# jerryli27/TwinGAN

Hardware: AMD Instinct MI355X
Metric: training images/sec (G+D step) at 256×256 final stage, 1/2/4/8 MI355X (higher is better)
Workload: dtype bf16; 1 GPU; TwinGAN 256x256 stage, batch 16 per GPU (configs[3]): E/G/2xD max_ch 256, UNet + per-domain instance norm + pixel norm, WGAN-GP, Adam; 1 step = G apply + D apply; global_batch=16, batch_per_gpu=16, parallelism=dp1, launch=hipGraph replay

## Files before the change

twingan_amd/csrc/reduce.hip:

```cpp
#include "tg_common.h"
#include "../../include/twingan_hip_optim.h"
#include "../../include/twingan_hip_summary.h"

namespace {

constexpr int MB_NMAX = 16;
template <typename T, int V>
struct alignas(sizeof(T) * V) MbVec {
  T e[V];
  __device__ __forceinline__ float get(int i) const { return (float)e[i]; }
  __device__ __forceinline__ void set(int i, float x) { e[i] = (T)x; }
};
template <typename T> constexpr int mb_v() { return 8 / (int)sizeof(T); }
template <typename T, int V> __device__ __forceinline__ MbVec<T, V> mb_ld(const T* p) {
  return *reinterpret_cast<const MbVec<T, V>*>(p);
}
template <typename T, int V> __device__ __forceinline__ void mb_st(T* p, const MbVec<T, V>& v) {
  *reinterpret_cast<MbVec<T, V>*>(p) = v;
}
template <typename T, int V>
__device__ __forceinline__ void mb_load_samples(const T* __restrict__ x, int n, int P, int p, MbVec<T, V> (&xv)[MB_NMAX]) {
#pragma unroll
  for (int i = 0; i < MB_NMAX; ++i) xv[i] = mb_ld<T, V>(x + (int64_t)(i < n ? i : n - 1) * P + p);
}


template <typename T, int U = 4>
__device__ __forceinline__ void mb_copy_with_stat(const T* __restrict__ src, T* __restrict__ out, int64_t nvec, int c,
                                                  int cpad, float val) {
  constexpr int V = Vec16<T>::N;
  const int cvp = cpad / V;
  for (int64_t i0 = threadIdx.x; i0 < nvec; i0 += (int64_t)blockDim.x * U) {
    Vec16<T> o[U];
#pragma unroll
    for (int u = 0; u < U; ++u) {
      int64_t i = i0 + (int64_t)u * blockDim.x;
      i = i < nvec ? i : nvec - 1;
      const int cb = (int)(i % cvp) * V;
      const int64_t px = i / cvp;
      if (cb < c) {
        o[u] = ldv(src + px * c + cb);
      } else {
#pragma unroll
        for (int j = 0; j < V; ++j) o[u].set(j, (cb + j == c) ? val : 0.f);
      }
    }
#pragma unroll
    for (int u = 0; u < U; ++u) {
      const int64_t i = i0 + (int64_t)u * blockDim.x;
      if (i < nvec) stv(out + (i / cvp) * cpad + (int)(i % cvp) * V, o[u]);
    }
  }
}

template <typename T>
__global__ __launch_bounds__(1024) void mbstd_fwd_kernel(const T* __restrict__ x, T* __restrict__ out,
                                                         float* __restrict__ stat, int n, int hw, int c, int cpad,
                                                         float eps) {
  __shared__ float red[16];
  const int P = hw * c;
  x += (int64_t)blockIdx.x * n * P;
  out += (int64_t)blockIdx.x * n * hw * cpad;
  if (stat) stat += blockIdx.x;
  float acc = 0.f;
  constexpr int V = mb_v<T>();
  if (P % V == 0 && n <= 32) {
    for (int p = threadIdx.x * V; p < P; p += blockDim.x * V) {
      float mu[V], var[V];
#pragma unroll
      for (int j = 0; j < V; ++j) mu[j] = var[j] = 0.f;
      if (n <= MB_NMAX) {
        MbVec<T, V> xs[MB_NMAX];
        mb_load_samples<T, V>(x, n, P, p, xs);
#pragma unroll
        for (int i = 0; i < MB_NMAX; ++i)
          if (i < n) {
#pragma unroll
            for (int j = 0; j < V; ++j) mu[j] += xs[i].get(j);
          }
#pragma unroll
        for (int j = 0; j < V; ++j) mu[j] /= (float)n;
#pragma unroll
        for (int i = 0; i < MB_NMAX; ++i)
          if (i < n) {
#pragma unroll
            for (int j = 0; j < V; ++j) {
              const float d = xs[i].get(j) - mu[j];
              var[j] = fmaf(d, d, var[j]);
            }
          }
      } else {
        for (int i = 0; i < n; ++i) {
          const MbVec<T, V> xv = mb_ld<T, V>(x + (int64_t)i * P + p);
#pragma unroll
          for (int j = 0; j < V; ++j) mu[j] += xv.get(j);
        }
#pragma unroll
        for (int j = 0; j < V; ++j) mu[j] /= (float)n;
        for (int i = 0; i < n; ++i) {
          const MbVec<T, V> xv = mb_ld<T, V>(x + (int64_t)i * P + p);
#pragma unroll
          for (int j = 0; j < V; ++j) {
            const float d = xv.get(j) - mu[j];
            var[j] = fmaf(d, d, var[j]);
          }
        }
      }
#pragma unroll
      for (int j = 0; j < V; ++j) acc += sqrtf(var[j] / (float)n + eps);
    }
  } else {
    for (int p = threadIdx.x; p < P; p += blockDim.x) {
      float mu = 0.f;
      for (int i = 0; i < n; ++i) mu += ld(x + (int64_t)i * P + p);
      mu /= (float)n;
      float var = 0.f;
      for (int i = 0; i < n; ++i) {
        const float d = ld(x + (int64_t)i * P + p) - mu;
        var = fmaf(d, d, var);
      }
      acc += sqrtf(var / (float)n + eps);
    }
  }
  const float val = block_sum(acc, red) / (float)P;
  if (threadIdx.x == 0 && stat) stat[0] = val;
  const int64_t total = (int64_t)n * hw * cpad;
  constexpr int V16 = Vec16<T>::N;
  if (c % V16 == 0 && cpad % V16 == 0) {
    mb_copy_with_stat<T, 9>(x, out, total / V16, c, cpad, val);
  } else {
    for (int64_t i = threadIdx.x; i < total; i += blockDim.x) {
      const int ch = (int)(i % cpad);
      const int64_t px = i / cpad;
      float v = 0.f;
      if (ch < c)
        v = ld(x + px * c + ch);
      else if (ch == c)
        v = val;
      st(out + i, v);
    }
  }
}

template <typename T>
__global__ __launch_bounds__(256) void mbstd_bwd_kernel(const T* __restrict__ gout, const T* __restrict__ x,
                                                        T* __restrict__ gx, int n, int hw, int c, int cpad, float eps) {
  __shared__ float red[16];
  const int P = hw * c;
  gout += (int64_t)blockIdx.x * n * hw * cpad;
  x += (int64_t)blockIdx.x * n * P;
  gx += (int64_t)blockIdx.x * n * P;
  constexpr int V = mb_v<T>();
  const bool fast = c % V == 0 && cpad % V == 0 && n <= MB_NMAX;
  MbVec<T, V> xs[MB_NMAX], gs[MB_NMAX];
  const int pstep = gridDim.y * blockDim.x * V;
  const int pfirst = (blockIdx.y * blockDim.x + threadIdx.x) * V;
  if (fast) {
    const int p = pfirst < P ? pfirst : 0;
    const int px = p / c, ch = p - px * c;
    mb_load_samples<T, V>(x, n, P, p, xs);
#pragma unroll
    for (int i = 0; i < MB_NMAX; ++i) gs[i] = mb_ld<T, V>(gout + ((int64_t)(i < n ? i : n - 1) * hw + px) * cpad + ch);
  }
  float acc = 0.f;
  for (int i = threadIdx.x; i < n * hw; i += blockDim.x) acc += ld(gout + (int64_t)i * cpad + c);
  const float G = block_sum(acc, red);
  if (fast) {
    for (int p = pfirst; p < P; p += pstep) {
      float mu[V], var[V], k[V];
      if (p != pfirst) {
        const int px = p / c, ch = p - px * c;
        mb_load_samples<T, V>(x, n, P, p, xs);
#pragma unroll
        for (int i = 0; i < MB_NMAX; ++i) gs[i] = mb_ld<T, V>(gout + ((int64_t)(i < n ? i : n - 1) * hw + px) * cpad + ch);
      }
#pragma unroll
      for (int j = 0; j < V; ++j) mu[j] = var[j] = 0.f;
#pragma unroll
      for (int i = 0; i < MB_NMAX; ++i)
        if (i < n) {
#pragma unroll
          for (int j = 0; j < V; ++j) mu[j] += xs[i].get(j);
        }
#pragma unroll
// ... 47 lines not shown
        const MbVec<T, V> xv = mb_ld<T, V>(x + (int64_t)i * P + p);
        const MbVec<T, V> gv = mb_ld<T, V>(gout + ((int64_t)i * hw + px) * cpad + ch);
        MbVec<T, V> o;
#pragma unroll
        for (int j = 0; j < V; ++j) o.set(j, gv.get(j) + k[j] * (xv.get(j) - mu[j]));
        mb_st<T, V>(gx + (int64_t)i * P + p, o);
      }
    }
    return;
  }
  for (int p = blockIdx.y * blockDim.x + threadIdx.x; p < P; p += gridDim.y * blockDim.x) {
    float mu = 0.f;
    for (int i = 0; i < n; ++i) mu += ld(x + (int64_t)i * P + p);
    mu /= (float)n;
    float var = 0.f;
    for (int i = 0; i < n; ++i) {
      const float d = ld(x + (int64_t)i * P + p) - mu;
      var = fmaf(d, d, var);
    }
    const float sigma = sqrtf(var / (float)n + eps);
    const float k = G / ((float)n * sigma * (float)P);
    const int px = p / c, ch = p - px * c;
    for (int i = 0; i < n; ++i) {
      const float d = ld(x + (int64_t)i * P + p) - mu;
      st(gx + (int64_t)i * P + p, ld(gout + ((int64_t)i * hw + px) * cpad + ch) + k * d);
    }
  }
}

template <typename T, int NTHR>
__global__ __launch_bounds__(NTHR) void mbstd_bwd_bwd_kernel(const T* __restrict__ v, const T* __restrict__ gout,
                                                            const T* __restrict__ x, T* __restrict__ ggout,
                                                            T* __restrict__ gx2, int n, int hw, int c, int cpad,
                                                            float eps) {
  __shared__ float red[16];
  const int P = hw * c;
  v += (int64_t)blockIdx.x * n * P;
  gout += (int64_t)blockIdx.x * n * hw * cpad;
  x += (int64_t)blockIdx.x * n * P;
  if (ggout) ggout += (int64_t)blockIdx.x * n * hw * cpad;
  if (gx2) gx2 += (int64_t)blockIdx.x * n * P;
  constexpr int V = mb_v<T>();
  const bool fast = P % V == 0 && n <= MB_NMAX;
  MbVec<T, V> xs[MB_NMAX], vs[MB_NMAX];
  const int pfirst = threadIdx.x * V;
  if (fast) {
    mb_load_samples<T, V>(x, n, P, pfirst < P ? pfirst : 0, xs);
    mb_load_samples<T, V>(v, n, P, pfirst < P ? pfirst : 0, vs);
  }
  float acc = 0.f;
  for (int i = threadIdx.x; i < n * hw; i += blockDim.x) acc += ld(gout + (int64_t)i * cpad + c);
  const float G = block_sum(acc, red);
  float tacc = 0.f;
  if (fast) {
    for (int p = pfirst; p < P; p += blockDim.x * V) {
      if (p != pfirst) {
        mb_load_samples<T, V>(x, n, P, p, xs);
        mb_load_samples<T, V>(v, n, P, p, vs);
      }
      float mu[V], vm[V], var[V], vc[V], sigma[V];
#pragma unroll
      for (int j = 0; j < V; ++j) mu[j] = vm[j] = var[j] = vc[j] = 0.f;
#pragma unroll
      for (int i = 0; i < MB_NMAX; ++i)
        if (i < n) {
#pragma unroll
          for (int j = 0; j < V; ++j) {
            mu[j] += xs[i].get(j);
            vm[j] += vs[i].get(j);
          }
        }
#pragma unroll
      for (int j = 0; j < V; ++j) {
        mu[j] /= (float)n;
        vm[j] /= (float)n;
      }
#pragma unroll
      for (int i = 0; i < MB_NMAX; ++i)
        if (i < n) {
#pragma unroll
          for (int j = 0; j < V; ++j) {
            const float d = xs[i].get(j) - mu[j];
            var[j] = fmaf(d, d, var[j]);
            vc[j] = fmaf(vs[i].get(j), d, vc[j]);
          }
        }
#pragma unroll
      for (int j = 0; j < V; ++j) {
        sigma[j] = sqrtf(var[j] / (float)n + eps);
        tacc += vc[j] / ((float)n * sigma[j] * (float)P);
      }
      if (gx2) {
        const float k = G / ((float)n * (float)P);
        float is[V], cf[V];
#pragma unroll
        for (int j = 0; j < V; ++j) {
          is[j] = 1.f / sigma[j];
          cf[j] = vc[j] * is[j] * is[j] * is[j] / (float)n;
        }
#pragma unroll
        for (int i = 0; i < MB_NMAX; ++i)
          if (i < n) {
            MbVec<T, V> o;
#pragma unroll
            for (int j = 0; j < V; ++j) {
              const float d = xs[i].get(j) - mu[j];
              o.set(j, k * ((vs[i].get(j) - vm[j]) * is[j] - cf[j] * d));
            }
            mb_st<T, V>(gx2 + (int64_t)i * P + p, o);
          }
      }
    }
  }
  for (int p = threadIdx.x; p < P && !fast; p += blockDim.x) {
    float mu = 0.f, vm = 0.f;
    for (int i = 0; i < n; ++i) {
      mu += ld(x + (int64_t)i * P + p);
      vm += ld(v + (int64_t)i * P + p);
    }
    mu /= (float)n;
    vm /= (float)n;
    float var = 0.f, vc = 0.f;
    for (int i = 0; i < n; ++i) {
      const float d = ld(x + (int64_t)i * P + p) - mu;
      var = fmaf(d, d, var);
      vc = fmaf(ld(v + (int64_t)i * P + p), d, vc);
    }
    const float sigma = sqrtf(var / (float)n + eps);
    tacc += vc / ((float)n * sigma * (float)P);
    if (gx2) {
      const float k = G / ((float)n * (float)P);
      for (int i = 0; i < n; ++i) {
        const float d = ld(x + (int64_t)i * P + p) - mu;
        const float vi = ld(v + (int64_t)i * P + p);
        st(gx2 + (int64_t)i * P + p, k * ((vi - vm) / sigma - vc * d / ((float)n * sigma * sigma * sigma)));
      }
    }
  }
  const float Tt = block_sum(tacc, red);
  if (ggout) {
    const int64_t total = (int64_t)n * hw * cpad;
    constexpr int V16 = Vec16<T>::N;
    if (c % V16 == 0 && cpad % V16 == 0) {
      mb_copy_with_stat<T, 9>(v, ggout, total / V16, c, cpad, Tt);
    } else {
      for (int64_t i = threadIdx.x; i < total; i += blockDim.x) {
        const int ch = (int)(i % cpad);
        const int64_t px = i / cpad;
        float o = 0.f;
        if (ch < c)
          o = ld(v + px * c + ch);
        else if (ch == c)
          o = Tt;
        st(ggout + i, o);
      }
    }
  }
}

template <typename T, int MODE, bool PART = false>
__global__ void sum_kernel(const T* __restrict__ x, const T* __restrict__ y, float* __restrict__ out, int64_t numel,
                           float scale, int direct = 0, int vec = 1) {
  __shared__ float red[8];
  constexpr int V = Vec16<T>::N;
  const int64_t nvec = vec ? numel / V : 0, stride = (int64_t)gridDim.x * blockDim.x;
  float acc = 0.f;
  for (int64_t i = (int64_t)blockIdx.x * blockDim.x + threadIdx.x; i < nvec; i += stride) {
    Vec16<T> a = ldv(x + i * V);
    if (MODE == 0) {
#pragma unroll
      for (int j = 0; j < V; ++j) acc += a.get(j);
    } else {
      Vec16<T> b = ldv(y + i * V);
#pragma unroll
      for (int j = 0; j < V; ++j) acc += fabsf(a.get(j) - b.get(j));
    }
  }
  for (int64_t i = nvec * V + (int64_t)blockIdx.x * blockDim.x + threadIdx.x; i < numel; i += stride)
    acc += MODE == 0 ? ld(x + i) : fabsf(ld(x + i) - ld(y + i));
  const float tot = block_sum(acc, red);
  if (threadIdx.x == 0) {
    if constexpr (PART) out[blockIdx.x] = tot;
    else if (direct) out[0] = tot * scale;
    else atomicAdd(out, tot * scale);
  }
}

__global__ void ordered_scalar_sum_kernel(const float* __restrict__ part, int n, float* __restrict__ out, float scale,
                                          int accumulate) {
  if (blockIdx.x || threadIdx.x) return;
  float t = 0.f;
  for (int i = 0; i < n; ++i) t += part[i];
  out[0] = accumulate ? out[0] + t * scale : t * scale;
}

__device__ __forceinline__ int nonfinite_bits(float x) {
  return (__builtin_bit_cast(uint32_t, x) & 0x7f800000u) == 0x7f800000u;
}
__device__ __forceinline__ float nan_where_nonfinite(float grad, float arg) {
  return nonfinite_bits(arg) ? __builtin_nanf("") : grad;
}

template <typename T>
__global__ void abs_diff_bwd_kernel(const T* __restrict__ a, const T* __restrict__ b, const float* __restrict__ gscale,
                                    T* __restrict__ ga, T* __restrict__ gb, int64_t numel, float scale) {
  const float g = (gscale ? gscale[0] : 1.f) * scale;
  for (int64_t i = (int64_t)blockIdx.x * blockDim.x + threadIdx.x; i < numel; i += (int64_t)gridDim.x * blockDim.x) {
    const float d = ld(a + i) - ld(b + i);
    const float s = nan_where_nonfinite(d > 0.f ? g : (d < 0.f ? -g : 0.f), d);
    if (ga) st(ga + i, s);
    if (gb) st(gb + i, -s);
  }
}

template <typename T>
__global__ void sample_sumsq_kernel(const T* __restrict__ x, float* __restrict__ out, int64_t per, int vec) {
  __shared__ float red[8];
  constexpr int V = Vec16<T>::N;
  const T* base = x + (int64_t)blockIdx.y * per;
  const int64_t nvec = vec ? per / V : 0, stride = (int64_t)gridDim.x * blockDim.x;
  float acc = 0.f;
  for (int64_t i = (int64_t)blockIdx.x * blockDim.x + threadIdx.x; i < nvec; i += stride) {
    Vec16<T> a = ldv(base + i * V);
#pragma unroll
    for (int j = 0; j < V; ++j) acc = fmaf(a.get(j), a.get(j), acc);
  }
  for (int64_t i = nvec * V + (int64_t)blockIdx.x * blockDim.x + threadIdx.x; i < per; i += stride) {
    const float a = ld(base + i);
    acc = fmaf(a, a, acc);
  }
  const float tot = block_sum(acc, red);
  if (threadIdx.x == 0) atomicAdd(out + blockIdx.y, tot);
}

__global__ void gp_penalty_kernel(const float* __restrict__ ss, float* __restrict__ loss, float* __restrict__ coef,
                                  int batch, float lambda) {
  __shared__ float red[8];
  float acc = 0.f;
  for (int b = threadIdx.x; b < batch; b += blockDim.x) {
    const float slope = sqrtf(ss[b]);
    const float d = slope - 1.f;
    acc += d * d;
    if (coef) coef[b] = slope == 0.f ? 0.f : lambda * 2.f * d / (slope * (float)batch);
  }
  const float tot = block_sum(acc, red);
  if (threadIdx.x == 0 && loss) loss[0] = lambda * tot / (float)batch;
}

__device__ __forceinline__ float pred_loss_f(float x, int mode, float a, float b) {
  if (mode == 1) {
    const float z = a + b * x;
    return z < 0.f ? 0.f : z;
  }
  if (mode == 2) return fmaxf(x, 0.f) - x * a + log1pf(expf(-fabsf(x)));
  if (mode == 3) return x * x;
  return x;
}
__device__ __forceinline__ float pred_loss_df_finite(float x, int mode, float a, float b) {
  if (mode == 1) return (a + b * x) > 0.f ? b : 0.f;
  if (mode == 2) return 1.f / (1.f + expf(-x)) - a;
  if (mode == 3) return 2.f * x;
  return 1.f;
}
__device__ __forceinline__ float pred_loss_df(float x, int mode, float a, float b) {
  return nan_where_nonfinite(pred_loss_df_finite(x, mode, a, b), x);
}
__global__ void pred_loss_fwd_kernel(const float* __restrict__ x, float* __restrict__ out, int n, int mode, float a,
                                     float b, float scale, int accumulate) {
  __shared__ float red[8];
  float acc = 0.f;
  for (int i = threadIdx.x; i < n; i += blockDim.x) acc += pred_loss_f(x[i], mode, a, b);
  const float tot = block_sum(acc, red);
  if (threadIdx.x == 0) out[0] = (accumulate ? out[0] : 0.f) + scale * tot;
}
__global__ void pred_loss_bwd_kernel(const float* __restrict__ x, const float* __restrict__ gscale, float* __restrict__ gx,
                                     int n, int mode, float a, float b, float scale) {
  const float g = (gscale ? gscale[0] : 1.f) * scale;
  for (int i = blockIdx.x * blockDim.x + threadIdx.x; i < n; i += gridDim.x * blockDim.x)
// ... 56 lines not shown
  for (int r = 0; r < b; ++r) {
    float dot = 0.f, se = 0.f, sp = 0.f;
    for (int c = threadIdx.x; c < d; c += 256) {
      const float x = e[(size_t)r * d + c], y = p[(size_t)r * d + c];
      dot = fmaf(x, y, dot);
      se = fmaf(x, x, se);
      sp = fmaf(y, y, sp);
    }
    dot = block_sum(dot, red);
    se = block_sum(se, red);
    sp = block_sum(sp, red);
    tot += 1.f - dot * rsqrtf(fmaxf(se, 1e-12f)) * rsqrtf(fmaxf(sp, 1e-12f));
  }
  if (threadIdx.x == 0) out[0] = tot * scale;
}

__global__ __launch_bounds__(256) void cosine_distance_bwd_kernel(const float* __restrict__ e, const float* __restrict__ p,
                                                                  const float* __restrict__ gscale, float* __restrict__ gp,
                                                                  int d, float scale) {
  __shared__ float red[4];
  const int r = blockIdx.x;
  float dot = 0.f, se = 0.f, sp = 0.f;
  for (int c = threadIdx.x; c < d; c += 256) {
    const float x = e[(size_t)r * d + c], y = p[(size_t)r * d + c];
    dot = fmaf(x, y, dot);
    se = fmaf(x, x, se);
    sp = fmaf(y, y, sp);
  }
  dot = block_sum(dot, red);
  se = block_sum(se, red);
  sp = block_sum(sp, red);
  const float ie = rsqrtf(fmaxf(se, 1e-12f)), ip = rsqrtf(fmaxf(sp, 1e-12f));
  const float cosv = dot * ie * ip, k = -scale * gscale[0];
  const bool clamped = sp < 1e-12f;
  for (int c = threadIdx.x; c < d; c += 256) {
    const float eh = e[(size_t)r * d + c] * ie, ph = p[(size_t)r * d + c] * ip;
    gp[(size_t)r * d + c] = k * (clamped ? eh * ip : (eh - ph * cosv) * ip);
  }
}

__global__ void var_from_sums_kernel(const float* __restrict__ s1, const float* __restrict__ ss, float* __restrict__ out,
                                     int batch, float inv_numel) {
  __shared__ float red[8];
  float acc = 0.f;
  for (int i = threadIdx.x; i < batch; i += blockDim.x) acc += ss[i];
  const float tot = block_sum(acc, red);
  if (threadIdx.x == 0) {
    const float m = s1[0] * inv_numel;
    const float v = tot * inv_numel - m * m;
    out[0] = v < 0.f ? 0.f : v;
  }
}

template <typename T>
__global__ void fc_fwd_kernel(const T* __restrict__ x, const float* __restrict__ w, const float* __restrict__ b,
                              float* __restrict__ y, int m, int n, int k) {
  const int64_t total = (int64_t)m * n;
  const int lane = threadIdx.x & 63;
  const int64_t w0 = ((int64_t)blockIdx.x * blockDim.x + threadIdx.x) >> 6, nw = ((int64_t)gridDim.x * blockDim.x) >> 6;
  for (int64_t i = w0; i < total; i += nw) {
    const int col = (int)(i % n), row = (int)(i / n);
    float acc = 0.f;
    for (int kk = lane; kk < k; kk += 64) acc = fmaf(ld(x + (int64_t)row * k + kk), w[(int64_t)kk * n + col], acc);
#pragma unroll
    for (int o = 32; o > 0; o >>= 1) acc += __shfl_xor(acc, o, 64);
    if (lane == 0) y[i] = acc + (b ? b[col] : 0.f);
  }
}
template <typename T>
__global__ void fc_bwd_kernel(const T* __restrict__ x, const float* __restrict__ w, const float* __restrict__ g,
                              T* __restrict__ gx, float* __restrict__ gw, float* __restrict__ gb, int m, int n, int k,
                              int acc_w, int acc_b) {
  const int kk = blockIdx.x * blockDim.x + threadIdx.x;
  if (kk < k) {
    for (int row = 0; gx && row < m; ++row) {
      float a = 0.f;
      for (int col = 0; col < n; ++col) a = fmaf(g[(int64_t)row * n + col], w[(int64_t)kk * n + col], a);
      st(gx + (int64_t)row * k + kk, a);
    }
    for (int col = 0; gw && col < n; ++col) {
      float a = 0.f;
      for (int row = 0; row < m; ++row) a = fmaf(ld(x + (int64_t)row * k + kk), g[(int64_t)row * n + col], a);
      gw[(int64_t)kk * n + col] = (acc_w ? gw[(int64_t)kk * n + col] : 0.f) + a;
    }
  }
  if (gb && kk < n) {
    float a = 0.f;
    for (int row = 0; row < m; ++row) a += g[(int64_t)row * n + kk];
    gb[kk] = (acc_b ? gb[kk] : 0.f) + a;
  }
}

__global__ void small_gemm_kernel(const float* __restrict__ a, const float* __restrict__ b, const float* __restrict__ bias,
                                  float* __restrict__ c, int m, int n, int k, int ta, int tb, int accumulate) {
  const int64_t total = (int64_t)m * n;
  for (int64_t i = (int64_t)blockIdx.x * blockDim.x + threadIdx.x; i < total; i += (int64_t)gridDim.x * blockDim.x) {
    const int col = (int)(i % n), row = (int)(i / n);
    float acc = 0.f;
    for (int kk = 0; kk < k; ++kk) {
      const float av = ta ? a[(int64_t)kk * m + row] : a[(int64_t)row * k + kk];
      const float bv = tb ? b[(int64_t)col * k + kk] : b[(int64_t)kk * n + col];
      acc = fmaf(av, bv, acc);
    }
    if (bias) acc += bias[col];
    c[i] = (accumulate ? c[i] : 0.f) + acc;
  }
}

__global__ void small_gemm_wave_kernel(const float* __restrict__ a, const float* __restrict__ b,
                                       const float* __restrict__ bias, float* __restrict__ c, int m, int n, int k, int ta,
                                       int tb, int accumulate) {
  const int64_t total = (int64_t)m * n;
  const int lane = threadIdx.x & 63;
  const int64_t w0 = ((int64_t)blockIdx.x * blockDim.x + threadIdx.x) >> 6, nw = ((int64_t)gridDim.x * blockDim.x) >> 6;
  for (int64_t i = w0; i < total; i += nw) {
    const int col = (int)(i % n), row = (int)(i / n);
    float acc = 0.f;
    for (int kk = lane; kk < k; kk += 64) {
      const float av = ta ? a[(int64_t)kk * m + row] : a[(int64_t)row * k + kk];
      const float bv = tb ? b[(int64_t)col * k + kk] : b[(int64_t)kk * n + col];
      acc = fmaf(av, bv, acc);
    }
    acc = wave_sum(acc);
    if (lane == 0) {
      if (bias) acc += bias[col];
      c[i] = (accumulate ? c[i] : 0.f) + acc;
    }
  }
}

__device__ __forceinline__ float adam_element(float th, float gi, float& m, float& v, float lr_t, float b1, float b2, float eps) {
  const float mi = fmaf(b1, m, (1.f - b1) * gi);
  const float vi = fmaf(b2, v, (1.f - b2) * gi * gi);
  m = mi;
  v = vi;
  return th - lr_t * mi / (sqrtf(vi) + eps);
}

__device__ __forceinline__ float ema_element(float avg, float var, float w) { return fmaf(-(avg - var), w, avg); }

template <bool VEC>
__device__ __forceinline__ void ema_span(float* __restrict__ avg, const float* __restrict__ var, int64_t numel, float w,
// ... 373 lines not shown
  }
  if ((tid & 63) == 0) red[tid >> 6] = SummaryPartial{acc.sum, acc.sumsq, acc.mn, acc.mx, acc.num, acc.zeros, acc.nonfinite, 0u};
  __syncthreads();
  if (tid == 0) {
    SummaryPartial r = red[0];
    for (int w = 1; w < SUM_THREADS / TG_WAVE; ++w) {
      r.sum += red[w].sum;
      r.sumsq += red[w].sumsq;
      r.mn = fminf(r.mn, red[w].mn);
      r.mx = fmaxf(r.mx, red[w].mx);
      r.num += red[w].num;
      r.zeros += red[w].zeros;
      r.nonfinite += red[w].nonfinite;
    }
    partials[b] = r;
  }
  uint32_t* dst = buckets + (size_t)j.out * TG_SUMMARY_BUCKETS;
  for (int i = tid; i < TG_SUMMARY_BUCKETS; i += SUM_THREADS) {
    const unsigned n = hist[i];
    if (n) atomicAdd(&dst[i], n);
  }
}

__global__ __launch_bounds__(64) void summary_finish_kernel(const SummaryJob* __restrict__ jobs, int njobs, int nout,
                                                            const SummaryPartial* __restrict__ partials,
                                                            TgSummaryStats* __restrict__ stats) {
  const int k = blockIdx.x * 64 + threadIdx.x;
  if (k >= njobs) return;
  const SummaryJob j = jobs[k];
  if (j.out >= nout) return;
  TgSummaryStats r{0.0, 0.0, SUM_FLT_MAX, -SUM_FLT_MAX, 0u, 0u, 0u, 0u};
  for (int b = j.block_begin; b < j.block_end; ++b) {
    const SummaryPartial p = partials[b];
    r.sum += p.sum;
    r.sum_squares += p.sumsq;
    r.min = fminf(r.min, p.mn);
    r.max = fmaxf(r.max, p.mx);
    r.num += p.num;
    r.zeros += p.zeros;
    r.nonfinite += p.nonfinite;
  }
  stats[j.out] = r;
}

}

extern "C" {

int tg_mbstd_fwd(const void* x, void* out, float* stat, int n, int groups, int hw, int c, int cpad, float eps, int dtype,
                 void* stream) {
  TG_CHECK(x && out && n > 0 && hw > 0 && c > 0 && cpad > c, TG_EINVAL, "tg_mbstd_fwd: bad arguments (cpad must exceed c)");
  TG_CHECK(groups > 0 && n % groups == 0, TG_EINVAL, "tg_mbstd_fwd: n (%d) not divisible by groups (%d)", n, groups);
  TG_DISPATCH_DTYPE(dtype, "tg_mbstd_fwd", {
    hipLaunchKernelGGL(mbstd_fwd_kernel<T>, dim3(groups), dim3(1024), 0, (hipStream_t)stream, (const T*)x, (T*)out, stat,
                       n / groups, hw, c, cpad, eps);
  });
  TG_LAUNCH_CHECK("tg_mbstd_fwd");
  return TG_OK;
}

int tg_mbstd_bwd(const void* gout, const void* x, void* gx, int n, int groups, int hw, int c, int cpad, float eps,
                 int dtype, void* stream) {
  TG_CHECK(gout && x && gx && n > 0 && hw > 0 && c > 0 && cpad > c, TG_EINVAL, "tg_mbstd_bwd: bad arguments");
  TG_CHECK(groups > 0 && n % groups == 0, TG_EINVAL, "tg_mbstd_bwd: n (%d) not divisible by groups (%d)", n, groups);
  TG_DISPATCH_DTYPE(dtype, "tg_mbstd_bwd", {
    int nsplit = (hw * c / mb_v<T>() + 255) / 256;
    if (nsplit < 1) nsplit = 1;
    if (nsplit > 8) nsplit = 8;
    hipLaunchKernelGGL(mbstd_bwd_kernel<T>, dim3(groups, nsplit), dim3(256), 0, (hipStream_t)stream, (const T*)gout, (const T*)x,
                       (T*)gx, n / groups, hw, c, cpad, eps);
  });
  TG_LAUNCH_CHECK("tg_mbstd_bwd");
  return TG_OK;
}

int tg_mbstd_bwd_bwd(const void* v, const void* gout, const void* x, void* ggout, void* gx2, int n, int groups, int hw, int c,
                     int cpad, float eps, int dtype, void* stream) {
  TG_CHECK(v && gout && x && n > 0 && hw > 0 && c > 0 && cpad > c, TG_EINVAL, "tg_mbstd_bwd_bwd: bad arguments");
  TG_CHECK(groups > 0 && n % groups == 0, TG_EINVAL, "tg_mbstd_bwd_bwd: n (%d) not divisible by groups (%d)", n, groups);
  TG_DISPATCH_DTYPE(dtype, "tg_mbstd_bwd_bwd", {
    constexpr int NTHR = sizeof(T) == 4 ? 512 : 1024;
    hipLaunchKernelGGL((mbstd_bwd_bwd_kernel<T, NTHR>), dim3(groups), dim3(NTHR), 0, (hipStream_t)stream, (const T*)v,
                       (const T*)gout, (const T*)x, (T*)ggout, (T*)gx2, n / groups, hw, c, cpad, eps);
  });
  TG_LAUNCH_CHECK("tg_mbstd_bwd_bwd");
  return TG_OK;
}

static int zero_unless(float* p, size_t bytes, int accumulate, hipStream_t s, const char* who) {
  if (!accumulate) return tg_zero_async(p, bytes, nullptr, 0, s);
  return TG_OK;
}

int tg_sum(const void* x, float* out, int64_t numel, float scale, int accumulate, int dtype, void* stream) {
  TG_CHECK(x && out && numel > 0, TG_EINVAL, "tg_sum: bad arguments");
  hipStream_t s = (hipStream_t)stream;
  TG_DISPATCH_DTYPE(dtype, "tg_sum", {
    const int blocks = exact_grid<T>() ? 1 : tg_grid_for(numel / Vec16<T>::N + 1, 256, 1024);
    const int direct = (blocks == 1 && !accumulate) ? 1 : 0;
    if (!direct) {
      int rc = zero_unless(out, sizeof(float), accumulate, s, "tg_sum");
      if (rc) return rc;
    }
    hipLaunchKernelGGL((sum_kernel<T, 0>), dim3(blocks), dim3(256), 0, s, (const T*)x, (const T*)nullptr, out, numel, scale, direct,
                       tg_aligned16(x));
  });
  TG_LAUNCH_CHECK("tg_sum");
  return TG_OK;
}

int tg_abs_diff_sum(const void* a, const void* b, float* out, int64_t numel, float scale, int accumulate, int dtype,
                    void* stream) {
  TG_CHECK(a && b && out && numel > 0, TG_EINVAL, "tg_abs_diff_sum: bad arguments");
  hipStream_t s = (hipStream_t)stream;
  TG_DISPATCH_DTYPE(dtype, "tg_abs_diff_sum", {
    const int blocks = exact_grid<T>() ? 1 : tg_grid_for(numel / Vec16<T>::N + 1, 256, 1024);
    const int direct = (blocks == 1 && !accumulate) ? 1 : 0;
    if (!direct) {
      int rc = zero_unless(out, sizeof(float), accumulate, s, "tg_abs_diff_sum");
      if (rc) return rc;
    }
    hipLaunchKernelGGL((sum_kernel<T, 1>), dim3(blocks), dim3(256), 0, s, (const T*)a, (const T*)b, out, numel, scale, direct,
                       tg_aligned16(a) && tg_aligned16(b));
  });
  TG_LAUNCH_CHECK("tg_abs_diff_sum");
  return TG_OK;
}

int tg_sum_ordered(const void* x, const void* y_or_null, float* out, int64_t numel, float scale, int accumulate, float* ws,
                   size_t ws_floats, int dtype, void* stream) {
  TG_CHECK(x && out && ws && ws_floats >= 1 && numel > 0, TG_EINVAL, "tg_sum_ordered: bad arguments");
  hipStream_t s = (hipStream_t)stream;
  int blocks = 0;
  TG_DISPATCH_DTYPE(dtype, "tg_sum_ordered", {
    blocks = tg_grid_for(numel / Vec16<T>::N + 1, 256, 512);
    if ((size_t)blocks > ws_floats) blocks = (int)ws_floats;
    if (y_or_null)
      hipLaunchKernelGGL((sum_kernel<T, 1, true>), dim3(blocks), dim3(256), 0, s, (const T*)x, (const T*)y_or_null, ws, numel, 1.f, 0,
                         tg_aligned16(x) && tg_aligned16(y_or_null));
    else
      hipLaunchKernelGGL((sum_kernel<T, 0, true>), dim3(blocks), dim3(256), 0, s, (const T*)x, (const T*)nullptr, ws, numel, 1.f, 0,
                         tg_aligned16(x));
  });
  hipLaunchKernelGGL(ordered_scalar_sum_kernel, dim3(1), dim3(64), 0, s, ws, blocks, out, scale, accumulate);
  TG_LAUNCH_CHECK("tg_sum_ordered");
  return TG_OK;
}

int tg_abs_diff_bwd(const void* a, const void* b, const float* gscale, void* ga, void* gb, int64_t numel, float scale,
                    int dtype, void* stream) {
  TG_CHECK(a && b && numel > 0 && (ga || gb), TG_EINVAL, "tg_abs_diff_bwd: bad arguments");
  TG_DISPATCH_DTYPE(dtype, "tg_abs_diff_bwd", {
    hipLaunchKernelGGL(abs_diff_bwd_kernel<T>, dim3(tg_grid_for(numel, 256)), dim3(256), 0, (hipStream_t)stream,
                       (const T*)a, (const T*)b, gscale, (T*)ga, (T*)gb, numel, scale);
  });
  TG_LAUNCH_CHECK("tg_abs_diff_bwd");
  return TG_OK;
}

int tg_sample_sumsq(const void* x, float* out, int batch, int64_t per, int dtype, void* stream) {
  TG_CHECK(x && out && batch > 0 && per > 0, TG_EINVAL, "tg_sample_sumsq: bad arguments");
  hipStream_t s = (hipStream_t)stream;
  int rc = zero_unless(out, (size_t)batch * sizeof(float), 0, s, "tg_sample_sumsq");
  if (rc) return rc;
  TG_DISPATCH_DTYPE(dtype, "tg_sample_sumsq", {
    const int chunks = exact_grid<T>() ? 1 : tg_grid_for(per / Vec16<T>::N + 1, 256, 64);
    const int vec = tg_aligned16(x) && (batch == 1 || per % Vec16<T>::N == 0);
    hipLaunchKernelGGL(sample_sumsq_kernel<T>, dim3(chunks, batch), dim3(256), 0, s, (const T*)x, out, per, vec);
  });
  TG_LAUNCH_CHECK("tg_sample_sumsq");
  return TG_OK;
}

int tg_gp_penalty(const float* sumsq, float* loss, float* coef, int batch, float lambda, void* stream) {
  TG_CHECK(sumsq && batch > 0, TG_EINVAL, "tg_gp_penalty: bad arguments");
  hipLaunchKernelGGL(gp_penalty_kernel, dim3(1), dim3(256), 0, (hipStream_t)stream, sumsq, loss, coef, batch, lambda);
  TG_LAUNCH_CHECK("tg_gp_penalty");
  return TG_OK;
}

int tg_pred_loss_fwd(const float* x, float* out, int n, int mode, float a, float b, float scale, int accumulate,
                     void* stream) {
  TG_CHECK(x && out && n > 0 && mode >= 0 && mode <= 3, TG_EINVAL, "tg_pred_loss_fwd: bad arguments");
  hipLaunchKernelGGL(pred_loss_fwd_kernel, dim3(1), dim3(256), 0, (hipStream_t)stream, x, out, n, mode, a, b, scale,
                     accumulate);
  TG_LAUNCH_CHECK("tg_pred_loss_fwd");
  return TG_OK;
}

int tg_pred_loss_bwd(const float* x, const float* gscale, float* gx, int n, int mode, float a, float b, float scale,
                     void* stream) {
  TG_CHECK(x && gx && n > 0 && mode >= 0 && mode <= 3, TG_EINVAL, "tg_pred_loss_bwd: bad arguments");
  hipLaunchKernelGGL(pred_loss_bwd_kernel, dim3(tg_grid_for(n, 256)), dim3(256), 0, (hipStream_t)stream, x, gscale, gx, n,
                     mode, a, b, scale);
  TG_LAUNCH_CHECK("tg_pred_loss_bwd");
  return TG_OK;
}

int tg_pred_losses_fwd(const float* pred, int group_size, int groups, const TgPredJob* jobs, int njobs, float* terms, int nterms,
                       void* stream) {
  TG_CHECK(pred && jobs && terms && group_size > 0 && groups > 0 && njobs > 0 && njobs <= PRED_MAX_JOBS && nterms > 0 &&
               nterms <= PRED_MAX_TERMS, TG_EINVAL, "tg_pred_losses_fwd: bad arguments (at most %d jobs, %d terms)", PRED_MAX_JOBS,
           PRED_MAX_TERMS);
  PredJobs pj;
  pj.n = njobs;
  for (int j = 0; j < njobs; ++j) {
    TG_CHECK(jobs[j].group >= 0 && jobs[j].group < groups && jobs[j].term >= 0 && jobs[j].term < nterms && jobs[j].mode >= 0 &&
                 jobs[j].mode <= 3, TG_EINVAL, "tg_pred_losses_fwd: job %d out of range", j);
    pj.j[j] = jobs[j];
  }
  hipLaunchKernelGGL(pred_losses_fwd_kernel, dim3(1), dim3(256), 0, (hipStream_t)stream, pred, group_size, pj, terms, nterms);
  TG_LAUNCH_CHECK("tg_pred_losses_fwd");
  return TG_OK;
}

int tg_pred_losses_bwd(const float* pred, int group_size, int groups, const TgPredJob* jobs, int njobs, const float* const* gterms,
                       int nterms, float* gpred, void* stream) {
  TG_CHECK(pred && jobs && gterms && gpred && group_size > 0 && groups > 0 && njobs > 0 && njobs <= PRED_MAX_JOBS && nterms > 0 &&
               nterms <= PRED_MAX_TERMS, TG_EINVAL, "tg_pred_losses_bwd: bad arguments");
// ... 29 lines not shown
                           void* stream) {
  TG_CHECK(expected && embedding && out && batch > 0 && dim > 0, TG_EINVAL, "tg_cosine_distance_fwd: bad arguments");
  hipLaunchKernelGGL(cosine_distance_fwd_kernel, dim3(1), dim3(256), 0, (hipStream_t)stream, expected, embedding, out, batch,
                     dim, weight / (float)batch);
  TG_LAUNCH_CHECK("tg_cosine_distance_fwd");
  return TG_OK;
}

int tg_cosine_distance_bwd(const float* expected, const float* embedding, const float* gscale, float* g_embedding, int batch,
                           int dim, float weight, void* stream) {
  TG_CHECK(expected && embedding && gscale && g_embedding && batch > 0 && dim > 0, TG_EINVAL,
           "tg_cosine_distance_bwd: bad arguments");
  hipLaunchKernelGGL(cosine_distance_bwd_kernel, dim3(batch), dim3(256), 0, (hipStream_t)stream, expected, embedding, gscale,
                     g_embedding, dim, weight / (float)batch);
  TG_LAUNCH_CHECK("tg_cosine_distance_bwd");
  return TG_OK;
}

int tg_var_from_sums(const float* sum, const float* sample_sumsq, float* out, int batch, int64_t numel, void* stream) {
  TG_CHECK(sum && sample_sumsq && out && batch > 0 && numel > 0, TG_EINVAL, "tg_var_from_sums: bad arguments");
  hipLaunchKernelGGL(var_from_sums_kernel, dim3(1), dim3(256), 0, (hipStream_t)stream, sum, sample_sumsq, out, batch,
                     1.0f / (float)numel);
  TG_LAUNCH_CHECK("tg_var_from_sums");
  return TG_OK;
}

int tg_small_gemm(const float* a, const float* b, const float* bias, float* c, int m, int n, int k, int ta, int tb,
                  int accumulate, void* stream) {
  TG_CHECK(a && b && c && m > 0 && n > 0 && k > 0, TG_EINVAL, "tg_small_gemm: bad arguments");
  if (k >= 32 && (int64_t)m * n <= 4096)
    hipLaunchKernelGGL(small_gemm_wave_kernel, dim3(tg_grid_for((int64_t)m * n * 64, 256)), dim3(256), 0,
                       (hipStream_t)stream, a, b, bias, c, m, n, k, ta, tb, accumulate);
  else
    hipLaunchKernelGGL(small_gemm_kernel, dim3(tg_grid_for((int64_t)m * n, 256)), dim3(256), 0, (hipStream_t)stream, a, b,
                       bias, c, m, n, k, ta, tb, accumulate);
  TG_LAUNCH_CHECK("tg_small_gemm");
  return TG_OK;
}

int tg_fc_fwd(const void* x, const float* w, const float* bias, float* y, int m, int n, int k, int dtype, void* stream) {
  TG_CHECK(x && w && y && m > 0 && n > 0 && k > 0, TG_EINVAL, "tg_fc_fwd: bad arguments");
  TG_DISPATCH_DTYPE(dtype, "tg_fc_fwd", {
    hipLaunchKernelGGL(fc_fwd_kernel<T>, dim3(tg_grid_for((int64_t)m * n * 64, 256)), dim3(256), 0, (hipStream_t)stream,
                       (const T*)x, w, bias, y, m, n, k);
  });
  TG_LAUNCH_CHECK("tg_fc_fwd");
  return TG_OK;
}

int tg_fc_bwd(const void* x, const float* w, const float* g, void* gx, float* gw, float* gb, int m, int n, int k, int acc_w,
              int acc_b, int dtype, void* stream) {
  TG_CHECK(x && w && g && (gx || gw || gb) && m > 0 && n > 0 && k > 0 && n <= k, TG_EINVAL, "tg_fc_bwd: bad arguments");
  TG_DISPATCH_DTYPE(dtype, "tg_fc_bwd", {
    hipLaunchKernelGGL(fc_bwd_kernel<T>, dim3(tg_grid_for(k, 64)), dim3(64), 0, (hipStream_t)stream, (const T*)x, w, g, (T*)gx,
                       gw, gb, m, n, k, acc_w, acc_b);
  });
  TG_LAUNCH_CHECK("tg_fc_bwd");
  return TG_OK;
}

int tg_adam_step(float* theta, const float* grad, float* m, float* v, void* theta_bf16, int64_t numel, float lr_t,
                 const float* lr_t_dev, float beta1, float beta2, float eps, float grad_scale, void* stream) {
  TG_CHECK(theta && grad && m && v && numel > 0, TG_EINVAL, "tg_adam_step: bad arguments");
  ApplyArgs a{theta, grad, m, v, numel, {lr_t, beta1, beta2, eps}, grad_scale};
  a.lr_t_dev = lr_t_dev;
  a.shadow = (bf16*)theta_bf16;
  return launch_apply<TG_OPT_ADAM>(a, stream, "tg_adam_step");
}

int tg_adam_ema_step(float* theta, const float* grad, float* m, float* v, float* avg, int64_t numel, const float* lr_t_dev,
                     float beta1, float beta2, float eps, float grad_scale, const float* w_dev, void* stream) {
  TG_CHECK(theta && grad && m && v && avg && lr_t_dev && w_dev, TG_EINVAL, "tg_adam_ema_step: null pointer");
  TG_CHECK(numel > 0, TG_EINVAL, "tg_adam_ema_step: numel must be positive (got %lld)", (long long)numel);
  return launch_apply<TG_OPT_ADAM>({theta, grad, m, v, numel, {0.f, beta1, beta2, eps}, grad_scale, nullptr, avg, w_dev, lr_t_dev},
                                   stream, "tg_adam_ema_step");
}

int tg_ema_update(float* avg, const float* var, int64_t numel, const float* w_dev, void* stream) {
  TG_CHECK(avg && var && w_dev, TG_EINVAL, "tg_ema_update: null pointer");
  TG_CHECK(numel > 0, TG_EINVAL, "tg_ema_update: numel must be positive (got %lld)", (long long)numel);
  if (tg_aligned16(avg) && tg_aligned16(var))
    hipLaunchKernelGGL(ema_kernel<true>, dim3(tg_grid_for((numel + 3) / 4, 256)), dim3(256), 0, (hipStream_t)stream, avg, var,
                       numel, w_dev);
  else
    hipLaunchKernelGGL(ema_kernel<false>, dim3(tg_grid_for(numel, 256)), dim3(256), 0, (hipStream_t)stream, avg, var, numel,
                       w_dev);
  TG_LAUNCH_CHECK("tg_ema_update");
  return TG_OK;
}

size_t tg_ema_table_bytes(int njobs) { return (size_t)(njobs > 0 ? njobs : 0) * sizeof(EmaJob); }

int tg_ema_table_fill(float* avg, const float* var, int64_t numel, int job, void* table_host, int32_t* total_blocks) {
  TG_CHECK(avg && var && table_host && total_blocks && job >= 0, TG_EINVAL, "tg_ema_table_fill: bad arguments");
  TG_CHECK(numel > 0, TG_EINVAL, "tg_ema_table_fill: numel must be positive (got %lld)", (long long)numel);
  const int64_t blocks = (numel + EMA_EPB - 1) / EMA_EPB;
  TG_CHECK(*total_blocks >= 0 && *total_blocks + blocks <= 0x7fffffff, TG_EINVAL, "tg_ema_table_fill: grid too large");
  EmaJob j;
  j.avg = avg;
  j.var = var;
  j.numel = numel;
  j.block_begin = *total_blocks;
  j.block_end = j.block_begin + (int)blocks;
  *total_blocks = j.block_end;
  ((EmaJob*)table_host)[job] = j;
  return TG_OK;
}
// ... 181 lines not shown
```

Baseline: 1049 images/sec.

## Split mbstd copies across grid.y, unroll reductions, and parallelize fc backward per element

Minibatch-stddev forward and double-backward kernels now launch extra blocks along grid.y. Each block redundantly recomputes the statistics and handles only a slice of the padded output copy and the per-sample gradient writes, which spreads a single-block-per-group copy over more CUs. The copy helper uses 32-bit index math with a smaller unroll. The sum and sum-of-squares reductions get an 8-way load unroll with fewer atomic blocks. The fc backward kernel is rewritten to give one thread per output element across the gx, gw and gb segments instead of one thread per k column looping over everything, with register-unrolled inner loops. The cost is duplicated stat computation per y-block and more launched blocks.

```diff
diff --git a/twingan_amd/csrc/reduce.hip b/twingan_amd/csrc/reduce.hip
--- a/twingan_amd/csrc/reduce.hip
+++ b/twingan_amd/csrc/reduce.hip
@@ -25,32 +25,45 @@
 }
 
 
-template <typename T, int U = 4>
+constexpr int MB_COPY_U = 3;
+template <typename T, int U, typename I>
+__device__ __forceinline__ void mb_copy_with_stat_as(const T* __restrict__ src, T* __restrict__ out, I nvec, int c,
+                                                     int cpad, float val) {
+  constexpr int V = Vec16<T>::N;
+  const I cvp = (I)(cpad / V), step = (I)gridDim.y * blockDim.x;
+  for (I i0 = (I)blockIdx.y * blockDim.x + threadIdx.x; i0 < nvec; i0 += step * U) {
+    Vec16<T> o[U];
+    I px[U];
+    int cb[U];
+#pragma unroll
+    for (int u = 0; u < U; ++u) {
+      I i = i0 + (I)u * step;
+      i = i < nvec ? i : nvec - 1;
+      px[u] = i / cvp;
+      cb[u] = (int)(i - px[u] * cvp) * V;
+      if (cb[u] < c) {
+        o[u] = ldv(src + (int64_t)px[u] * c + cb[u]);
+      } else {
+#pragma unroll
+        for (int j = 0; j < V; ++j) o[u].set(j, (cb[u] + j == c) ? val : 0.f);
+      }
+    }
+#pragma unroll
+    for (int u = 0; u < U; ++u)
+      if (i0 + (I)u * step < nvec) stv(out + (int64_t)px[u] * cpad + cb[u], o[u]);
+  }
+}
+template <typename T, int U = MB_COPY_U>
 __device__ __forceinline__ void mb_copy_with_stat(const T* __restrict__ src, T* __restrict__ out, int64_t nvec, int c,
                                                   int cpad, float val) {
-  constexpr int V = Vec16<T>::N;
-  const int cvp = cpad / V;
-  for (int64_t i0 = threadIdx.x; i0 < nvec; i0 += (int64_t)blockDim.x * U) {
-    Vec16<T> o[U];
-#pragma unroll
-    for (int u = 0; u < U; ++u) {
-      int64_t i = i0 + (int64_t)u * blockDim.x;
-      i = i < nvec ? i : nvec - 1;
-      const int cb = (int)(i % cvp) * V;
-      const int64_t px = i / cvp;
-      if (cb < c) {
-        o[u] = ldv(src + px * c + cb);
-      } else {
-#pragma unroll
-        for (int j = 0; j < V; ++j) o[u].set(j, (cb + j == c) ? val : 0.f);
-      }
-    }
-#pragma unroll
-    for (int u = 0; u < U; ++u) {
-      const int64_t i = i0 + (int64_t)u * blockDim.x;
-      if (i < nvec) stv(out + (i / cvp) * cpad + (int)(i % cvp) * V, o[u]);
-    }
-  }
+  if (nvec < (int64_t)1 << 30) mb_copy_with_stat_as<T, U, uint32_t>(src, out, (uint32_t)nvec, c, cpad, val);
+  else mb_copy_with_stat_as<T, U, int64_t>(src, out, nvec, c, cpad, val);
+}
+template <typename T> static int mb_copy_split(int n_per_group, int hw, int cpad, int threads) {
+  const int64_t nvec = (int64_t)n_per_group * hw * cpad / Vec16<T>::N;
+  const int64_t per = (int64_t)threads * MB_COPY_U;
+  const int64_t ny = (nvec + per - 1) / per;
+  return ny < 1 ? 1 : ny > 8 ? 8 : (int)ny;
 }
 
 template <typename T>
@@ -123,13 +136,13 @@
     }
   }
   const float val = block_sum(acc, red) / (float)P;
-  if (threadIdx.x == 0 && stat) stat[0] = val;
+  if (threadIdx.x == 0 && blockIdx.y == 0 && stat) stat[0] = val;
   const int64_t total = (int64_t)n * hw * cpad;
   constexpr int V16 = Vec16<T>::N;
   if (c % V16 == 0 && cpad % V16 == 0) {
-    mb_copy_with_stat<T, 9>(x, out, total / V16, c, cpad, val);
+    mb_copy_with_stat<T>(x, out, total / V16, c, cpad, val);
   } else {
-    for (int64_t i = threadIdx.x; i < total; i += blockDim.x) {
+    for (int64_t i = (int64_t)blockIdx.y * blockDim.x + threadIdx.x; i < total; i += (int64_t)gridDim.y * blockDim.x) {
       const int ch = (int)(i % cpad);
       const int64_t px = i / cpad;
       float v = 0.f;
@@ -283,6 +296,8 @@
   for (int i = threadIdx.x; i < n * hw; i += blockDim.x) acc += ld(gout + (int64_t)i * cpad + c);
   const float G = block_sum(acc, red);
   float tacc = 0.f;
+  unsigned mine = 0;
+  for (int i = blockIdx.y; i < MB_NMAX; i += gridDim.y) mine |= 1u << i;
   if (fast) {
     for (int p = pfirst; p < P; p += blockDim.x * V) {
       if (p != pfirst) {
@@ -331,7 +346,7 @@
         }
 #pragma unroll
         for (int i = 0; i < MB_NMAX; ++i)
-          if (i < n) {
+          if (i < n && (mine >> i & 1u)) {
             MbVec<T, V> o;
 #pragma unroll
             for (int j = 0; j < V; ++j) {
@@ -361,7 +376,7 @@
     tacc += vc / ((float)n * sigma * (float)P);
     if (gx2) {
       const float k = G / ((float)n * (float)P);
-      for (int i = 0; i < n; ++i) {
+      for (int i = blockIdx.y; i < n; i += gridDim.y) {
         const float d = ld(x + (int64_t)i * P + p) - mu;
         const float vi = ld(v + (int64_t)i * P + p);
         st(gx2 + (int64_t)i * P + p, k * ((vi - vm) / sigma - vc * d / ((float)n * sigma * sigma * sigma)));
@@ -373,9 +388,9 @@
     const int64_t total = (int64_t)n * hw * cpad;
     constexpr int V16 = Vec16<T>::N;
     if (c % V16 == 0 && cpad % V16 == 0) {
-      mb_copy_with_stat<T, 9>(v, ggout, total / V16, c, cpad, Tt);
+      mb_copy_with_stat<T>(v, ggout, total / V16, c, cpad, Tt);
     } else {
-      for (int64_t i = threadIdx.x; i < total; i += blockDim.x) {
+      for (int64_t i = (int64_t)blockIdx.y * blockDim.x + threadIdx.x; i < total; i += (int64_t)gridDim.y * blockDim.x) {
         const int ch = (int)(i % cpad);
         const int64_t px = i / cpad;
         float o = 0.f;
@@ -389,6 +404,8 @@
   }
 }
 
+constexpr int RED_U = 8;
+constexpr int RED_ATOMIC_BLOCKS = 256;
 template <typename T, int MODE, bool PART = false>
 __global__ void sum_kernel(const T* __restrict__ x, const T* __restrict__ y, float* __restrict__ out, int64_t numel,
                            float scale, int direct = 0, int vec = 1) {
@@ -396,16 +413,20 @@
   constexpr int V = Vec16<T>::N;
   const int64_t nvec = vec ? numel / V : 0, stride = (int64_t)gridDim.x * blockDim.x;
   float acc = 0.f;
-  for (int64_t i = (int64_t)blockIdx.x * blockDim.x + threadIdx.x; i < nvec; i += stride) {
-    Vec16<T> a = ldv(x + i * V);
-    if (MODE == 0) {
-#pragma unroll
-      for (int j = 0; j < V; ++j) acc += a.get(j);
-    } else {
-      Vec16<T> b = ldv(y + i * V);
-#pragma unroll
-      for (int j = 0; j < V; ++j) acc += fabsf(a.get(j) - b.get(j));
-    }
+  for (int64_t i0 = (int64_t)blockIdx.x * blockDim.x + threadIdx.x; i0 < nvec; i0 += stride * RED_U) {
+    Vec16<T> a[RED_U], b[RED_U];
+#pragma unroll
+    for (int u = 0; u < RED_U; ++u) {
+      const int64_t i = i0 + u * stride < nvec ? i0 + u * stride : nvec - 1;
+      a[u] = ldv(x + i * V);
+      if (MODE != 0) b[u] = ldv(y + i * V);
+    }
+#pragma unroll
+    for (int u = 0; u < RED_U; ++u)
+      if (i0 + u * stride < nvec) {
+#pragma unroll
+        for (int j = 0; j < V; ++j) acc += MODE == 0 ? a[u].get(j) : fabsf(a[u].get(j) - b[u].get(j));
+      }
   }
   for (int64_t i = nvec * V + (int64_t)blockIdx.x * blockDim.x + threadIdx.x; i < numel; i += stride)
     acc += MODE == 0 ? ld(x + i) : fabsf(ld(x + i) - ld(y + i));
@@ -451,10 +472,16 @@
   const T* base = x + (int64_t)blockIdx.y * per;
   const int64_t nvec = vec ? per / V : 0, stride = (int64_t)gridDim.x * blockDim.x;
   float acc = 0.f;
-  for (int64_t i = (int64_t)blockIdx.x * blockDim.x + threadIdx.x; i < nvec; i += stride) {
-    Vec16<T> a = ldv(base + i * V);
-#pragma unroll
-    for (int j = 0; j < V; ++j) acc = fmaf(a.get(j), a.get(j), acc);
+  for (int64_t i0 = (int64_t)blockIdx.x * blockDim.x + threadIdx.x; i0 < nvec; i0 += stride * RED_U) {
+    Vec16<T> a[RED_U];
+#pragma unroll
+    for (int u = 0; u < RED_U; ++u) a[u] = ldv(base + (i0 + u * stride < nvec ? i0 + u * stride : nvec - 1) * V);
+#pragma unroll
+    for (int u = 0; u < RED_U; ++u)
+      if (i0 + u * stride < nvec) {
+#pragma unroll
+        for (int j = 0; j < V; ++j) acc = fmaf(a[u].get(j), a[u].get(j), acc);
+      }
   }
   for (int64_t i = nvec * V + (int64_t)blockIdx.x * blockDim.x + threadIdx.x; i < per; i += stride) {
     const float a = ld(base + i);
@@ -617,6 +644,7 @@
   }
 }
 
+constexpr int FC_U = 16;
 template <typename T>
 __global__ void fc_fwd_kernel(const T* __restrict__ x, const float* __restrict__ w, const float* __restrict__ b,
                               float* __restrict__ y, int m, int n, int k) {
@@ -636,23 +664,67 @@
 __global__ void fc_bwd_kernel(const T* __restrict__ x, const float* __restrict__ w, const float* __restrict__ g,
                               T* __restrict__ gx, float* __restrict__ gw, float* __restrict__ gb, int m, int n, int k,
                               int acc_w, int acc_b) {
-  const int kk = blockIdx.x * blockDim.x + threadIdx.x;
-  if (kk < k) {
-    for (int row = 0; gx && row < m; ++row) {
-      float a = 0.f;
-      for (int col = 0; col < n; ++col) a = fmaf(g[(int64_t)row * n + col], w[(int64_t)kk * n + col], a);
-      st(gx + (int64_t)row * k + kk, a);
-    }
-    for (int col = 0; gw && col < n; ++col) {
-      float a = 0.f;
-      for (int row = 0; row < m; ++row) a = fmaf(ld(x + (int64_t)row * k + kk), g[(int64_t)row * n + col], a);
-      gw[(int64_t)kk * n + col] = (acc_w ? gw[(int64_t)kk * n + col] : 0.f) + a;
-    }
-  }
-  if (gb && kk < n) {
+  const int bx = gx ? (int)(((int64_t)m * k + blockDim.x - 1) / blockDim.x) : 0;
+  const int bw = gw ? (int)(((int64_t)k * n + blockDim.x - 1) / blockDim.x) : 0;
+  int b = blockIdx.x;
+  if (b < bx) {
+    const int64_t i = (int64_t)b * blockDim.x + threadIdx.x;
+    if (i >= (int64_t)m * k) return;
+    const int row = (int)(i / k), kk = (int)(i - (int64_t)row * k);
+    const float* gr = g + (int64_t)row * n;
+    const float* wr = w + (int64_t)kk * n;
     float a = 0.f;
-    for (int row = 0; row < m; ++row) a += g[(int64_t)row * n + kk];
-    gb[kk] = (acc_b ? gb[kk] : 0.f) + a;
+    for (int c0 = 0; c0 < n; c0 += FC_U) {
+      float gv[FC_U], wv[FC_U];
+#pragma unroll
+      for (int u = 0; u < FC_U; ++u) {
+        const int col = c0 + u < n ? c0 + u : n - 1;
+        gv[u] = gr[col];
+        wv[u] = wr[col];
+      }
+#pragma unroll
+      for (int u = 0; u < FC_U; ++u)
+        if (c0 + u < n) a = fmaf(gv[u], wv[u], a);
+    }
+    st(gx + i, a);
+    return;
+  }
+  b -= bx;
+  if (b < bw) {
+    const int64_t i = (int64_t)b * blockDim.x + threadIdx.x;
+    if (i >= (int64_t)k * n) return;
+    const int kk = (int)(i / n), col = (int)(i - (int64_t)kk * n);
+    const float prior = acc_w ? gw[i] : 0.f;
+    float a = 0.f;
+    for (int r0 = 0; r0 < m; r0 += FC_U) {
+      float xv[FC_U], gv[FC_U];
+#pragma unroll
+      for (int u = 0; u < FC_U; ++u) {
+        const int row = r0 + u < m ? r0 + u : m - 1;
+        xv[u] = ld(x + (int64_t)row * k + kk);
+        gv[u] = g[(int64_t)row * n + col];
+      }
+#pragma unroll
+      for (int u = 0; u < FC_U; ++u)
+        if (r0 + u < m) a = fmaf(xv[u], gv[u], a);
+    }
+    gw[i] = prior + a;
+    return;
+  }
+  b -= bw;
+  const int col = b * blockDim.x + threadIdx.x;
+  if (gb && col < n) {
+    const float prior = acc_b ? gb[col] : 0.f;
+    float a = 0.f;
+    for (int r0 = 0; r0 < m; r0 += FC_U) {
+      float gv[FC_U];
+#pragma unroll
+      for (int u = 0; u < FC_U; ++u) gv[u] = g[(int64_t)(r0 + u < m ? r0 + u : m - 1) * n + col];
+#pragma unroll
+      for (int u = 0; u < FC_U; ++u)
+        if (r0 + u < m) a += gv[u];
+    }
+    gb[col] = prior + a;
   }
 }
 
@@ -1132,8 +1204,8 @@
   TG_CHECK(x && out && n > 0 && hw > 0 && c > 0 && cpad > c, TG_EINVAL, "tg_mbstd_fwd: bad arguments (cpad must exceed c)");
   TG_CHECK(groups > 0 && n % groups == 0, TG_EINVAL, "tg_mbstd_fwd: n (%d) not divisible by groups (%d)", n, groups);
   TG_DISPATCH_DTYPE(dtype, "tg_mbstd_fwd", {
-    hipLaunchKernelGGL(mbstd_fwd_kernel<T>, dim3(groups), dim3(1024), 0, (hipStream_t)stream, (const T*)x, (T*)out, stat,
-                       n / groups, hw, c, cpad, eps);
+    hipLaunchKernelGGL(mbstd_fwd_kernel<T>, dim3(groups, mb_copy_split<T>(n / groups, hw, cpad, 1024)), dim3(1024), 0,
+                       (hipStream_t)stream, (const T*)x, (T*)out, stat, n / groups, hw, c, cpad, eps);
   });
   TG_LAUNCH_CHECK("tg_mbstd_fwd");
   return TG_OK;
@@ -1160,8 +1232,9 @@
   TG_CHECK(groups > 0 && n % groups == 0, TG_EINVAL, "tg_mbstd_bwd_bwd: n (%d) not divisible by groups (%d)", n, groups);
   TG_DISPATCH_DTYPE(dtype, "tg_mbstd_bwd_bwd", {
     constexpr int NTHR = sizeof(T) == 4 ? 512 : 1024;
-    hipLaunchKernelGGL((mbstd_bwd_bwd_kernel<T, NTHR>), dim3(groups), dim3(NTHR), 0, (hipStream_t)stream, (const T*)v,
-                       (const T*)gout, (const T*)x, (T*)ggout, (T*)gx2, n / groups, hw, c, cpad, eps);
+    hipLaunchKernelGGL((mbstd_bwd_bwd_kernel<T, NTHR>), dim3(groups, mb_copy_split<T>(n / groups, hw, cpad, NTHR)), dim3(NTHR), 0,
+                       (hipStream_t)stream, (const T*)v, (const T*)gout, (const T*)x, (T*)ggout, (T*)gx2, n / groups, hw, c,
+                       cpad, eps);
   });
   TG_LAUNCH_CHECK("tg_mbstd_bwd_bwd");
   return TG_OK;
@@ -1176,7 +1249,7 @@
   TG_CHECK(x && out && numel > 0, TG_EINVAL, "tg_sum: bad arguments");
   hipStream_t s = (hipStream_t)stream;
   TG_DISPATCH_DTYPE(dtype, "tg_sum", {
-    const int blocks = exact_grid<T>() ? 1 : tg_grid_for(numel / Vec16<T>::N + 1, 256, 1024);
+    const int blocks = exact_grid<T>() ? 1 : tg_grid_for(numel / Vec16<T>::N + 1, 256, RED_ATOMIC_BLOCKS);
     const int direct = (blocks == 1 && !accumulate) ? 1 : 0;
     if (!direct) {
       int rc = zero_unless(out, sizeof(float), accumulate, s, "tg_sum");
@@ -1194,7 +1267,7 @@
   TG_CHECK(a && b && out && numel > 0, TG_EINVAL, "tg_abs_diff_sum: bad arguments");
   hipStream_t s = (hipStream_t)stream;
   TG_DISPATCH_DTYPE(dtype, "tg_abs_diff_sum", {
-    const int blocks = exact_grid<T>() ? 1 : tg_grid_for(numel / Vec16<T>::N + 1, 256, 1024);
+    const int blocks = exact_grid<T>() ? 1 : tg_grid_for(numel / Vec16<T>::N + 1, 256, RED_ATOMIC_BLOCKS);
     const int direct = (blocks == 1 && !accumulate) ? 1 : 0;
     if (!direct) {
       int rc = zero_unless(out, sizeof(float), accumulate, s, "tg_abs_diff_sum");
@@ -1244,7 +1317,8 @@
   int rc = zero_unless(out, (size_t)batch * sizeof(float), 0, s, "tg_sample_sumsq");
   if (rc) return rc;
   TG_DISPATCH_DTYPE(dtype, "tg_sample_sumsq", {
-    const int chunks = exact_grid<T>() ? 1 : tg_grid_for(per / Vec16<T>::N + 1, 256, 64);
+    const int chunk_cap = batch >= RED_ATOMIC_BLOCKS ? 1 : RED_ATOMIC_BLOCKS / batch < 64 ? RED_ATOMIC_BLOCKS / batch : 64;
+    const int chunks = exact_grid<T>() ? 1 : tg_grid_for(per / Vec16<T>::N + 1, 256, chunk_cap);
     const int vec = tg_aligned16(x) && (batch == 1 || per % Vec16<T>::N == 0);
     hipLaunchKernelGGL(sample_sumsq_kernel<T>, dim3(chunks, batch), dim3(256), 0, s, (const T*)x, out, per, vec);
   });
@@ -1380,7 +1454,9 @@
               int acc_b, int dtype, void* stream) {
   TG_CHECK(x && w && g && (gx || gw || gb) && m > 0 && n > 0 && k > 0 && n <= k, TG_EINVAL, "tg_fc_bwd: bad arguments");
   TG_DISPATCH_DTYPE(dtype, "tg_fc_bwd", {
-    hipLaunchKernelGGL(fc_bwd_kernel<T>, dim3(tg_grid_for(k, 64)), dim3(64), 0, (hipStream_t)stream, (const T*)x, w, g, (T*)gx,
+    const int64_t blocks = (gx ? ((int64_t)m * k + 255) / 256 : 0) + (gw ? ((int64_t)k * n + 255) / 256 : 0) + (gb ? (n + 255) / 256 : 0);
+    TG_CHECK(blocks <= INT32_MAX, TG_EINVAL, "tg_fc_bwd: m * k (%lld) too large for one launch", (long long)m * k);
+    hipLaunchKernelGGL(fc_bwd_kernel<T>, dim3((unsigned)blocks), dim3(256), 0, (hipStream_t)stream, (const T*)x, w, g, (T*)gx,
                        gw, gb, m, n, k, acc_w, acc_b);
   });
   TG_LAUNCH_CHECK("tg_fc_bwd");
```

Result: no change. 1053 images/sec (median of 6 runs) (+0.4%).
